# aliyun/heif-decoder-lib

Hardware: AMD Instinct MI355X
Metric: megapixels/sec HEIC grid->RGB24 (higher is better)
Workload: dtype u8

## Files before the change

### heif-decoder-lib_amd/csrc/chain.hip

```cpp
#include "recon_common.h"

#include <stdlib.h>
#include <atomic>
#include <map>
#include <memory>
#include <mutex>
#include <new>
#include <utility>

#include "hm_internal.h"

namespace {

#ifdef HM_CHAIN_TIMING
#define HM_T_DECL unsigned long long t_prev = __builtin_amdgcn_s_memtime(); unsigned int t_acc[6] = {0, 0, 0, 0, 0, 0}, t_part[4] = {0, 0, 0, 0}; int t_in_svc = 0; (void)t_part; (void)t_in_svc
#if HM_CHAIN_TIMING == 2
#define HM_T_LAP(i) (void)t_prev
#define HM_T_COUNT(i) t_acc[i] += 64
#else
#define HM_T_LAP(i) do { if (HM_CHAIN_TIMING != 4) { const unsigned long long t_now = __builtin_amdgcn_s_memtime(); t_acc[i] += (unsigned int)(t_now - t_prev); t_prev = t_now; } } while (0)
#define HM_T_COUNT(i)
#endif
#if HM_CHAIN_TIMING == 4
#define HM_T_SVC_BEGIN() do { t_prev = __builtin_amdgcn_s_memtime(); t_in_svc = 1; } while (0)
// ... 53 lines not shown
  int rows_per_wave, split_kinds, bands_per_pic;
  int passes;
  int ring;
  int spin_limit;
  int test_stall;
  int early;
};
constexpr int SYNC_TICKET = 0, SYNC_PROGRESS = 8;
constexpr int SPIN_LIMIT = 1 << 20;

__device__ __forceinline__ int g_of(int lane) { return lane >> 4; }
template <int CTRL>
__device__ __forceinline__ int dpp(int v) { return __builtin_amdgcn_update_dpp(0, v, CTRL, 0xF, 0xF, false); }
constexpr int DPP_ROW_ROR(int n) { return 0x120 | n; }
constexpr int DPP_ROW_SHR(int n) { return 0x110 | n; }

enum { ST_START = 0, ST_RUN = 1, ST_DONE = 2 };

typedef uint32_t c_u32x4 __attribute__((ext_vector_type(4)));
typedef uint32_t c_u32x2 __attribute__((ext_vector_type(2)));

#ifndef HM_WPE_ONE_CHAIN
#define HM_WPE_ONE_CHAIN 5
#endif
#ifndef HM_WPE_CTB64
#define HM_WPE_CTB64 4
#endif
template <typename Pix, int LOG2_CTB, int MODE>
constexpr int chain_waves_per_simd = (sizeof(Pix) == 1 && MODE == 0) ? (LOG2_CTB <= 5 ? 5 : HM_WPE_CTB64) :
                                     ((MODE >= 3 && !(sizeof(Pix) == 2 && LOG2_CTB == 6)) ? HM_WPE_ONE_CHAIN : 4);
// ... 519 lines not shown
      uint32_t run[2], big[2];
#pragma unroll
      for (int c = 0; c < 2; c++) {
        const uint32_t q = of_chain(gq, c), r = of_chain(gr, c);
        run[c] = (uint32_t)__builtin_ctz(~q | (1u << SUBX));
        big[c] = (uint32_t)__builtin_ctz(~((r & ~q) >> run[c]));
      }
      const uint32_t my_run = g == 0 ? run[0] : run[1], my_big = g == 0 ? big[0] : big[1];
      quad = (uint32_t)my_off < my_run;
      m_quad = ballot(quad);
      s_big = ballot((uint32_t)my_off >= my_run && (uint32_t)my_off < my_run + my_big);
      n_exec = (int)(my_run + my_big);
      n_sub = (int)(run[0] > run[1] ? run[0] : run[1]);
    }
    (void)m_quad;
    const unsigned long long s_bres = s_big & ballot((op.y & (OP_CBF | (3u << OP_L2_SHIFT))) == (OP_CBF | (1u << OP_L2_SHIFT)));

    HM_T_LAP(1);
#if defined(HM_Q_PROBE) && (HM_Q_PROBE & 2048)
    if (s_bres && n_pics < 0) {
#else
    if (s_bres) {
#endif
      auto big_res = [&](int gg) -> uint32_t {
        uint32_t idx = (uint32_t)__builtin_amdgcn_readlane((int)op.z, gg * 16) + (uint32_t)lane;
        idx = idx < res_last ? idx : res_last;
        return (uint32_t)(int)resid[idx];
      };
      uint32_t sb_lo = (uint32_t)s_bres, sb_hi = (uint32_t)(s_bres >> 32);
      asm volatile("" : "+s"(sb_lo), "+s"(sb_hi));
      if (sb_lo & 0xFFFFu) bres0 = big_res(0);
// ... 81 lines not shown
      HM_T_COUNT(4);
      const int src = bg * 16;
      const uint32_t ox = (uint32_t)__builtin_amdgcn_readlane((int)op.x, src), oy = (uint32_t)__builtin_amdgcn_readlane((int)op.y, src);
      const uint32_t oz = (uint32_t)__builtin_amdgcn_readlane((int)op.z, src), ow = (uint32_t)__builtin_amdgcn_readlane((int)op.w, src);
      const uint32_t s_gb = (uint32_t)__builtin_amdgcn_readlane((int)gb_off, src), s_tl = (uint32_t)__builtin_amdgcn_readlane((int)tl_off, src);
      const int mode = (int)(oy & OP_MODE_MASK), c = (int)((oy >> OP_C_SHIFT) & 3), log2 = 2 + (int)((oy >> OP_L2_SHIFT) & 3);
      const int path = (int)((oy >> OP_PATH_SHIFT) & 7);
#ifdef HM_D_SKIP
      if ((HM_D_SKIP >> (path != PATH_GEN ? path : 4 + log2)) & 1) continue;
#endif
#if defined(HM_Q_PROBE) && (HM_Q_PROBE & 512)
      const bool cbf = false;
#else
      const bool cbf = (oy & OP_CBF) != 0;
#endif
      const int P = c == 0 ? P0 : P1;
      Pix* const gb = reinterpret_cast<Pix*>(lds + s_gb);
      Pix* const lp = gb + (ox & 0xFFFF);
      const Pix* const tp = reinterpret_cast<const Pix*>(lds + ((oy & OP_LINE) ? s_tl : s_gb)) + (ox >> 16) + 1;
      Pix* const dst = lp + 1;
      const GLOBAL_AS int16_t* const gres = resid + oz;
      const int maxv = (1 << bd) - 1;

      HM_MARK("D_setup_end");
      auto block = [&](auto l2c, auto which) {
        constexpr int L2 = decltype(l2c)::value, WHICH = decltype(which)::value;
        int ln = lane;
        asm volatile("" : "+v"(ln));
        int res_s = 0, res_t[4] = {0, 0, 0, 0};
        const bool pairs = sizeof(Pix) == 1 && L2 >= 4 && WHICH != PATH_B4 && mode >= 2 && mode != 10 && mode != 26;
#ifdef HM_PAIRS_PRE
        uint32_t res_p[2] = {0, 0};
        if (cbf && pairs && L2 == 4) {
#pragma unroll
          for (int t = 0; t < 2; t++) res_p[t] = pairs8_residual<4>(mode >= 18, ln, t, gres);
        }
        else
#endif
        if (cbf && !pairs) {
          if (L2 == 2) {
            const int s_ri = __builtin_amdgcn_readlane((int)ri_me, src);
            const int s_chain = PAIRS ? bg & ((1 << NCL) - 1) : ((CAN_LATE && late) ? bg & 2 : bg);
            res_s = (int)(rres_all + s_chain * (RING * 16) + (s_ri & (RING - 1)) * 16)[ln & 15];
          }
          else if (L2 == 3) {
            uint32_t b = bg == 0 ? bres0 : (bg == 1 ? bres1 : (bg == 2 ? bres2 : bres3));
            asm volatile("" : "+v"(b));
            res_s = (int)b;
          }
          else if (L2 == 4) {
#pragma unroll
            for (int t = 0; t < 4; t++) res_t[t] = (int)gres[ln + 64 * t];
          }
        }
        auto emit = [&](int p, int x, int y, int v) {
          if (cbf) {
            int r;
            if (L2 <= 3) r = res_s;
            else if (L2 == 4) {
              const int t = rfl(p >> 6);
              r = t == 0 ? res_t[0] : (t == 1 ? res_t[1] : (t == 2 ? res_t[2] : res_t[3]));
            }
            else r = (int)gres[p];
            v = clip3i(0, maxv, v + r);
          }
          dst[mul24(y, P) + x] = (Pix)v;
        };
        Blk<Pix> B;
        B.mode = mode; B.c = c; B.bd = bd; B.log2 = L2; B.tskip = 0; B.qp = 0; B.n_coeff = 0; B.P = P;
        const bool smoothed = L2 != 2 && c == 0 && ((filter_mode_mask(L2) >> mode) & 1);
#if !defined(HM_Q_PROBE) || !(HM_Q_PROBE & 4)
        if (false) {}
        else if (WHICH == PATH_I16) {
// ... 3 lines not shown
          const int j = ln - 32;
          const int p = R(j), p_end = R(32);
          int pf = p;
          if (smoothed) {
            const int pm = dpp<0x138>(p);
            int pp = dpp<0x130>(p);
            pp = ln == 63 ? p_end : pp;
            pf = j == -32 ? p : (pm + 2 * p + pp + 2) >> 2;
          }
          int16_t* const bc = l_bA + 64;
          bc[j] = (int16_t)pf;
          if (ln == 0) bc[32] = (int16_t)p_end;
          WAVE_SYNC();
          if constexpr (sizeof(Pix) == 1 && L2 == 4) {
#ifdef HM_PAIRS_PRE
            if (pairs) predict_pairs8<4, true>(mode, bc, tab, ln, cbf, gres, reinterpret_cast<uint8_t*>(dst), P, res_p);
#else
            if (pairs) predict_pairs8<4, false>(mode, bc, tab, ln, cbf, gres, reinterpret_cast<uint8_t*>(dst), P);
#endif
            else predict_emit<Pix, L2>(B, RefArray{bc}, tab, ln, emit);
          }
          else predict_emit<Pix, L2>(B, RefArray{bc}, tab, ln, emit);
        }
        else if (WHICH == PATH_B4) {
          const uint32_t avail = ((ow & OPW_LEFT) ? 0xF0u : 0u) | (((ow >> OPW_BL_SHIFT) & 15) ? 0x0Fu : 0u) | ((ow & OPW_TL) ? 0x100u : 0u) |
                                 ((ow & OPW_TOP) ? 0x1E00u : 0u) | (((ow >> OPW_TR_SHIFT) & 15) ? 0x1E000u : 0u);
          const int b = ln < 16 ? ln : 16;
          const uint32_t lower = avail & ((1u << b) - 1u);
          const int first = avail ? (int)__builtin_ctz(avail) : 0;
          const int from = ((avail >> b) & 1u) ? b : (lower ? 31 - (int)__builtin_clz(lower) : first);
          const int j = from - 8;
          const Pix* const ql = lp + mul24_raw(-j - 1, P);
          const Pix* const qt = tp + (j - 1);
// ... 6 lines not shown
        }
        else {
          constexpr uint32_t nT = 1u << L2;
          B.info = L2 | (c << HM_TU_CIDX_SHIFT) | ((ow & OPW_TL) ? HM_TU_AVAIL_TL : 0);
          B.aBL = (int)(((ow >> OPW_BL_SHIFT) & 15) << 2); B.aTR = (int)(((ow >> OPW_TR_SHIFT) & 15) << 2);
          B.avail = ((ow & OPW_LEFT) ? nT : 0u) | ((uint32_t)B.aBL << 8) | ((ow & OPW_TOP) ? nT << 16 : 0u) | ((uint32_t)B.aTR << 24);
          B.x0 = (int)((ow >> 6) & 0x3C); B.y0 = (int)((ow >> 10) & 0x3C);
          B.u = gb + (c == 2 ? cr_off : 0);
          B.top = reinterpret_cast<const Pix*>(lds + s_tl) + (c == 2 ? Wc + 4 : 0);
#if !defined(HM_Q_PROBE) || !(HM_Q_PROBE & 16)
          make_border<Pix, L2>(B, l_bA, strong, ln);
          WAVE_SYNC();
          if constexpr (sizeof(Pix) == 1 && L2 >= 4) {
            if (pairs) {
#ifdef HM_PAIRS_PRE
              if constexpr (L2 == 4) predict_pairs8<4, true>(mode, l_bA + 64, tab, ln, cbf, gres, reinterpret_cast<uint8_t*>(dst), P, res_p);
              else
#endif
              predict_pairs8<L2, false>(mode, l_bA + 64, tab, ln, cbf, gres, reinterpret_cast<uint8_t*>(dst), P);
            }
            else predict_emit<Pix, L2>(B, RefArray{l_bA + 64}, tab, ln, emit);
          }
          else predict_emit<Pix, L2>(B, RefArray{l_bA + 64}, tab, ln, emit);
#endif
        }
#endif
        if (L2 >= 4) __builtin_amdgcn_s_waitcnt(0x0F70);
        WAVE_SYNC();
        HM_MARK("D_pred_end");
      };
#if defined(HM_Q_PROBE) && (HM_Q_PROBE & 256)
      if (path == PATH_F8A) continue;
#endif
#if !defined(HM_Q_PROBE) || !(HM_Q_PROBE & 128)
// ... 14 lines not shown
        }
        else {
          const int inv = inv_angle_of(mode);
          const int k0 = k + 1, k1 = k + 2;
          const int q0 = -((mul24(k0, inv) + 128) >> 8), q1 = -((mul24(k1, inv) + 128) >> 8);
          const int j0 = k0 >= 0 ? k0 : q0, j1 = k1 >= 0 ? k1 : q1;
          auto at = [&](int j, bool main_side) -> int {
            const Pix* const qm = vert ? tp + imin_(j - 1, nT1) : lp + mul24(imin_(j - 1, nL1), P);
            const Pix* const qs = vert ? lp + mul24(imin_(-j - 1, nL1), P) : tp + imin_(-j - 1, nT1);
            return *(main_side ? qm : qs);
          };
          r0 = vert ? at(j0, j0 >= 0) : at(j0, j0 > 0);
          r1 = vert ? at(j1, j1 >= 0) : at(j1, j1 > 0);
        }
        int v = blend32(f, r0, r1);
        if (cbf) {
          uint32_t b = bg == 0 ? bres0 : (bg == 1 ? bres1 : (bg == 2 ? bres2 : bres3));
          asm volatile("" : "+v"(b));
          v = clip3i(0, maxv, v + (int)b);
        }
        dst[mul24(y, P) + x] = (Pix)v;
        WAVE_SYNC();
        continue;
      }
      else if (path == PATH_F8O) {
        int ln = lane;
        asm volatile("" : "+v"(ln));
        const int x = ln & 7, y = ln >> 3;
        const int nL1 = (int)((oy >> OP_NL1_SHIFT) & 63), nT1 = (int)((oy >> OP_NT1_SHIFT) & 63);
        const int t = tp[x], l = lp[mul24(y, P)];
        int v;
        if (mode == 0) v = planar_sample<3>(x, y, l, t, tp[imin_(8, nT1)], lp[mul24(imin_(8, nL1), P)]);
        else if (mode == 1) {
          int s2 = ln < 8 ? t : (ln < 16 ? (int)lp[mul24(ln - 8, P)] : 0);
          s2 += dpp<DPP_ROW_ROR(8)>(s2);
// ... 6 lines not shown
            const int dc3 = mad24_k<3>(dc, 2);
            v = y == 0 ? (t + dc3) >> 2 : v;
            v = x == 0 ? (l + dc3) >> 2 : v;
            v = (x | y) == 0 ? (l + 2 * dc + t + 2) >> 2 : v;
          }
        }
        else {
          const bool vert = mode == 26;
          v = vert ? t : l;
          if (c == 0) {
            const int corner = tp[-1];
            const int gq = vert ? (int)tp[0] + ((l - corner) >> 1) : (int)lp[0] + ((t - corner) >> 1);
            v = (vert ? x == 0 : y == 0) ? clip3i(0, maxv, gq) : v;
          }
        }
        if (cbf) {
          uint32_t b = bg == 0 ? bres0 : (bg == 1 ? bres1 : (bg == 2 ? bres2 : bres3));
          asm volatile("" : "+v"(b));
          v = clip3i(0, maxv, v + (int)b);
        }
        dst[mul24(y, P) + x] = (Pix)v;
        WAVE_SYNC();
        continue;
      }
      else if (path == PATH_S8) {
        int ln = lane;
        asm volatile("" : "+v"(ln));
        const int nL1 = (int)((oy >> OP_NL1_SHIFT) & 63), nT1 = (int)((oy >> OP_NT1_SHIFT) & 63);
        const int j = ln < 32 ? ln - 16 : 16;
        const Pix* const ql = lp + mul24_raw(imin_(-j - 1, nL1), P);
        const Pix* const qt = tp + imin_(j - 1, nT1);
        const int p = *(j < 0 ? ql : qt);
        const int pm = dpp<0x138>(p), pp = dpp<0x130>(p);
        const int pf = (j == -16 || j == 16) ? p : (pm + 2 * p + pp + 2) >> 2;
        int16_t* const bc = l_bA + 64;
        if (ln <= 32) bc[j] = (int16_t)pf;
        WAVE_SYNC();
        const int x = ln & 7, y = ln >> 3;
        int v;
        if (mode == 0) v = planar_sample<3>(x, y, bc[-1 - y], bc[1 + x], bc[9], bc[-9]);
        else v = bc[mode == 34 ? x + y + 2 : (mode == 2 ? -(x + y + 2) : x - y)];
        if (cbf) {
          uint32_t b = bg == 0 ? bres0 : (bg == 1 ? bres1 : (bg == 2 ? bres2 : bres3));
          asm volatile("" : "+v"(b));
          v = clip3i(0, maxv, v + (int)b);
        }
        dst[mul24(y, P) + x] = (Pix)v;
        WAVE_SYNC();
        continue;
      }
#endif
#if defined(HM_Q_PROBE) && (HM_Q_PROBE & 96)
      {
        const bool sm = log2 == 3 && c == 0 && ((filter_mode_mask(3) >> mode) & 1);
        const bool fast = log2 <= 3 && !sm && (oy & OP_INTERIOR);
        if (((HM_Q_PROBE & 32) && !fast) || ((HM_Q_PROBE & 64) && fast)) continue;
      }
#endif
      typedef std::integral_constant<int, PATH_GEN> gen_t;
      if (path == PATH_I16) block(std::integral_constant<int, 4>(), std::integral_constant<int, PATH_I16>());
      else if (path == PATH_B4) block(std::integral_constant<int, 2>(), std::integral_constant<int, PATH_B4>());
// ... 550 lines not shown
```

### heif-decoder-lib_amd/csrc/recon_common.h

```cpp
#ifndef HM_RECON_COMMON_H
#define HM_RECON_COMMON_H

#include <hip/hip_runtime.h>
#include <stdint.h>
#include <type_traits>

#include "hm_device.h"

namespace {

#define WAVE_SYNC()                                          \
  do {                                                       \
    __builtin_amdgcn_fence(__ATOMIC_ACQ_REL, "wavefront");  \
    __builtin_amdgcn_wave_barrier();                         \
  } while (0)

__device__ __forceinline__ int clip3i(int lo, int hi, int v) { return v < lo ? lo : (v > hi ? hi : v); }
__device__ __forceinline__ int iabs_(int v) { return v < 0 ? -v : v; }
__device__ __forceinline__ int imin_(int a, int b) { return a < b ? a : b; }
__device__ __forceinline__ int mul24(int a, int b) { return __mul24(a, b); }
__device__ __forceinline__ int mul24_raw(int a, int b)
{
  int d;
  asm("v_mul_i32_i24 %0, %1, %2" : "=v"(d) : "v"(a), "v"(b));
// ... 58 lines not shown
  return -(int)(((ad <= 4 ? K1 : K2) >> (16 * ((ad - 1) & 3))) & 0xFFFF);
}
namespace angle_check {
constexpr int kAngle[35] = {0, 0, 32, 26, 21, 17, 13, 9, 5, 2, 0, -2, -5, -9, -13, -17, -21, -26, -32, -26, -21, -17, -13, -9, -5, -2, 0, 2, 5, 9, 13, 17, 21, 26, 32};
constexpr int kInv[15] = {-4096, -1638, -910, -630, -482, -390, -315, -256, -315, -390, -482, -630, -910, -1638, -4096};
constexpr bool same()
{
  for (int m = 2; m < 35; m++)
    if (intra_angle_of(m) != kAngle[m]) return false;
  for (int m = 11; m <= 25; m++)
    if (inv_angle_of(m) != kInv[m - 11]) return false;
  return true;
}
static_assert(same(), "intra_angle_of / inv_angle_of must reproduce Tables 8-4 / 8-5");
}
__constant__ int c_level_scale[6] = {40, 45, 51, 57, 64, 72};
__constant__ int8_t c_dst[4][4] = {{29, 55, 74, 84}, {74, 74, 0, -74}, {84, -29, -74, 55}, {55, -84, 74, -29}};
__constant__ int8_t c_dct_mag[33] = {64, 90, 90, 90, 89, 88, 87, 85, 83, 82, 80, 78, 75, 73, 70, 67, 64,
                                     61, 57, 54, 50, 46, 43, 38, 36, 31, 25, 22, 18, 13, 9, 4, 0};

#define GLOBAL_AS __attribute__((address_space(1)))
template <typename T>
__device__ __forceinline__ const GLOBAL_AS T* gptr(const void* p) { return (const GLOBAL_AS T*)(uintptr_t)p; }
template <typename T>
__device__ __forceinline__ GLOBAL_AS T* gptr_w(void* p) { return (GLOBAL_AS T*)(uintptr_t)p; }

constexpr int BIG_BYTES = 2048 + 1024 + 16;
constexpr int UPAD = 4;

template <typename Pix>
struct Blk {
  Pix* u;
  const Pix* top;
  int P;
// ... 259 lines not shown
    });
    }
  }
}
template <int L2>
__device__ __forceinline__ uint32_t pairs8_residual(bool vert, int lane, int t, const GLOBAL_AS int16_t* gres)
{
  constexpr int nT = 1 << L2;
  const int q = lane + 64 * t;
  const int x = vert ? (q & (nT / 2 - 1)) << 1 : q & (nT - 1), y = vert ? q >> (L2 - 1) : (q >> L2) << 1;
  if (vert) return *reinterpret_cast<const GLOBAL_AS uint32_t*>(gres + (x + (y << L2)));
  return (uint32_t)(uint16_t)gres[x + (y << L2)] | ((uint32_t)(uint16_t)gres[x + ((y + 1) << L2)] << 16);
}
template <int L2, bool PRE = false>
__device__ __forceinline__ void predict_pairs8(int mode, const int16_t* bc, const int16_t* tab, int lane, bool cbf, const GLOBAL_AS int16_t* gres, uint8_t* dst, int P,
                                               const uint32_t* pre = nullptr)
{
  constexpr int nT = 1 << L2, TRIPS = nT * nT / 128;
  typedef short s16x2_t __attribute__((ext_vector_type(2)));
  typedef unsigned short u16x2_t __attribute__((ext_vector_type(2)));
  const int angle = __builtin_amdgcn_readfirstlane((int)tab[mode]);
  const int inv = __builtin_amdgcn_readfirstlane((int)tab[35 + mode]);
  const bool vert = mode >= 18;
  auto ref = [&](int k) -> uint32_t {
    const int a = k >= 0 ? k : -((mul24(k, inv) + 128) >> 8);
    return (uint32_t)(uint16_t)bc[vert ? a : -a];
  };
  auto ref_pos = [&](int k) -> uint32_t { return (uint32_t)(uint16_t)bc[vert ? k : -k]; };
  auto trip = [&](int t) {
    const int q = lane + 64 * t;
    const int major = vert ? q >> (L2 - 1) : q & (nT - 1);
    const int m0 = vert ? (q & (nT / 2 - 1)) << 1 : (q >> L2) << 1;
    const int tt = mul24(major + 1, angle);
    const int k0 = m0 + (tt >> 5) + 1;
    const uint32_t f = (uint32_t)(tt & 31);
    uint32_t r0, r1, r2;
    if (angle > 0) { r0 = ref_pos(k0); r1 = ref_pos(k0 + 1); r2 = ref_pos(k0 + 2); }
    else { r0 = ref(k0); r1 = ref(k0 + 1); r2 = ref(k0 + 2); }
    const uint32_t A = r0 | (r1 << 16), B = r1 | (r2 << 16);
    const uint32_t w1 = f | (f << 16), w0 = 0x00200020u - w1;
    u16x2_t v = __builtin_bit_cast(u16x2_t, A) * __builtin_bit_cast(u16x2_t, w0) + __builtin_bit_cast(u16x2_t, B) * __builtin_bit_cast(u16x2_t, w1) + (u16x2_t)(16);
    v = v >> (u16x2_t)(5);
    const int x = vert ? m0 : major, y = vert ? major : m0;
    if (cbf) {
      uint32_t rr;
      if constexpr (PRE) rr = pre[t];
      else rr = pairs8_residual<L2>(vert, lane, t, gres);
      s16x2_t s = __builtin_bit_cast(s16x2_t, v) + __builtin_bit_cast(s16x2_t, rr);
      s = __builtin_elementwise_min(__builtin_elementwise_max(s, (s16x2_t)(0)), (s16x2_t)(255));
      v = __builtin_bit_cast(u16x2_t, s);
    }
    const uint32_t vw = __builtin_bit_cast(uint32_t, v);
    uint8_t* const o = dst + mul24(y, P) + x;
    if (vert) *reinterpret_cast<uint16_t*>(o) = (uint16_t)((vw & 0xFFu) | ((vw >> 8) & 0xFF00u));
    else { o[0] = (uint8_t)vw; o[P] = (uint8_t)(vw >> 16); }
  };
  if constexpr (TRIPS <= 2) {
#pragma unroll
    for (int t = 0; t < TRIPS; t++) trip(t);
  }
  else {
// ... 25 lines not shown
  return g;
}

constexpr uint32_t OP_MODE_MASK = 63u;
constexpr int OP_C_SHIFT = 6, OP_L2_SHIFT = 8;
constexpr uint32_t OP_CBF = 1u << 10, OP_INTERIOR = 1u << 11, OP_LINE = 1u << 13;
constexpr uint32_t OP_FAR = 1u << 26;
constexpr uint32_t OP_FAST8 = 1u << 12;
constexpr int OP_PATH_SHIFT = 27;
enum { PATH_GEN = 0,
       PATH_F8A = 1,
       PATH_F8O = 2,
       PATH_S8 = 3,
       PATH_I16 = 4,
       PATH_B4 = 5 };
constexpr uint32_t OP_SPECIAL = 1u << 31;
constexpr int OP_NL1_SHIFT = 14, OP_NT1_SHIFT = 20;
constexpr uint32_t OPW_LEFT = 1u << 16, OPW_TOP = 1u << 17, OPW_TL = 1u << 18;
constexpr int OPW_BL_SHIFT = 19, OPW_TR_SHIFT = 23;
typedef uint32_t mop_u32x4 __attribute__((ext_vector_type(4)));
__device__ __forceinline__ mop_u32x4 make_micro_op(uint32_t r0, unsigned a_left, unsigned a_top, unsigned a_tl, uint32_t aBL4, uint32_t aTR4, uint32_t qpy,
                                                   int Pk, int cr_off, int Wc, uint32_t roff)
{
  const int x4 = (int)(r0 & 15), y4 = (int)((r0 >> 4) & 15);
  const uint32_t info = (r0 >> 8) & 0xFF;
  const int l2 = (int)(info & HM_TU_LOG2_MASK), c = (int)((info >> HM_TU_CIDX_SHIFT) & 3);
  const uint32_t mode = (r0 >> 16) & OP_MODE_MASK;
  const bool cbf = (info & HM_TU_CBF) != 0;
  const int nT = 1 << l2;
  const bool left = a_left != 0, top = a_top != 0, tl = a_tl != 0;
// ... 200 lines not shown
```

### heif-decoder-lib_amd/csrc/residual.hip

```cpp
#include <cstdio>
#include <cstdlib>

#include "recon_common.h"
#include "hm_avail.h"

#include "hm_internal.h"

namespace {

constexpr int R_WAVES = 4;
constexpr int R_TABLES_SMALL = 1024 + 256 + 128;
constexpr int R_STAGE = 256;
constexpr int R_WAVE = 2048 + 1024 + 4 * 16 * 4 + R_STAGE * 4;

template <int CTRL>
__device__ __forceinline__ int rdpp(int v) { return __builtin_amdgcn_update_dpp(0, v, CTRL, 0xF, 0xF, false); }
constexpr int R_ROW_ROR(int n) { return 0x120 | n; }
constexpr int R_QUAD_BCAST(int k) { return k | (k << 2) | (k << 4) | (k << 6); }

typedef short r_s16x2 __attribute__((ext_vector_type(2)));
typedef uint32_t r_u32x4 __attribute__((ext_vector_type(4)));
typedef uint32_t r_u32x2 __attribute__((ext_vector_type(2)));
__device__ __forceinline__ int rdot2(uint32_t a, uint32_t b, int acc)
{
// ... 13 lines not shown
  v += rdpp_m<0x114, 0xF>(v);
  v += rdpp_m<0x118, 0xF>(v);
  v += rdpp_m<0x142, 0xA>(v);
  v += rdpp_m<0x143, 0xC>(v);
  return v;
}

template <int L2>
struct BigGeom {
  static constexpr int nT = 1 << L2;
  static constexpr int MT_STRIDE = nT + 4;
};
constexpr int R_MT16 = 16 * BigGeom<4>::MT_STRIDE * 2, R_MT32 = 32 * BigGeom<5>::MT_STRIDE * 2;
constexpr int R_TABLES = R_TABLES_SMALL + R_MT16 + R_MT32;
static_assert(R_TABLES % 16 == 0, "the waves' blocks are read 16 bytes at a time");
__device__ __forceinline__ int wave_max3(int v)
{
  int m = 0;
#pragma unroll
  for (int b = 2; b >= 0; b--) {
    const int t = m | (1 << b);
    if (ballot(v >= t)) m = t;
  }
  return m;
}
template <int L2, typename Levels>
__device__ __forceinline__ void big_residual(int16_t* coeff, int16_t* tmp, const int16_t* mt, const int16_t* tab, Levels cf,
                                             int n_coeff, int qP, int bit_depth, GLOBAL_AS int16_t* __restrict__ out, int lane)
{
  constexpr int nT = 1 << L2, log2 = L2, MS = BigGeom<L2>::MT_STRIDE;
// ... 60 lines not shown
#define HM_R_WPE 7
#endif
#ifndef HM_R_SKIP
#define HM_R_SKIP 0
#endif
#define HM_R_ATTR __attribute__((amdgpu_waves_per_eu(HM_R_WPE, HM_R_WPE)))
__global__ __launch_bounds__(R_WAVES * 64) HM_R_ATTR void k_residual(const hm_dev_pic* __restrict__ pics, int n_pics, int max_ctb_h, int segs)
{
  extern __shared__ __attribute__((aligned(16))) uint8_t lds[];
  const int tid = threadIdx.x, lane = tid & 63, wave = rfl(tid >> 6);
  int8_t* const dct = reinterpret_cast<int8_t*>(lds);
  int16_t* const tab = reinterpret_cast<int16_t*>(lds + 1024);
  uint32_t* const w8 = reinterpret_cast<uint32_t*>(lds + 1024 + 256);
  int16_t* const mt16 = reinterpret_cast<int16_t*>(lds + R_TABLES_SMALL);
  int16_t* const mt32 = reinterpret_cast<int16_t*>(lds + R_TABLES_SMALL + R_MT16);
  for (int i = tid; i < 1024; i += R_WAVES * 64) {
    const int k = i >> 5, n = i & 31;
    const int m = (k * (2 * n + 1)) & 127;
    int v;
    if (k == 0) v = 64;
    else if (m <= 32) v = c_dct_mag[m];
    else if (m <= 64) v = -c_dct_mag[64 - m];
    else if (m <= 96) v = -c_dct_mag[m - 64];
    else v = c_dct_mag[128 - m];
    dct[i] = (int8_t)v;
  }
  for (int i = tid; i < 92; i += R_WAVES * 64) {
    int v = 0;
    if (i >= 70 && i < 76) v = c_level_scale[i - 70];
    else if (i >= 76) v = c_dst[(i - 76) >> 2][(i - 76) & 3];
    tab[i] = (int16_t)v;
  }
  uint8_t* const wbase = lds + R_TABLES + (size_t)wave * R_WAVE;
  int16_t* const coeff = reinterpret_cast<int16_t*>(wbase);
  int16_t* const tmp = reinterpret_cast<int16_t*>(wbase + 2048);
  int* const slots = reinterpret_cast<int*>(wbase + 2048 + 1024);
  uint32_t* const lvl = reinterpret_cast<uint32_t*>(wbase + 2048 + 1024 + 4 * 16 * 4);
  for (int i = lane; i < 1024; i += 64) coeff[i] = 0;
  slots[lane] = 0;
  __syncthreads();
  for (int t = tid; t < 32; t += R_WAVES * 64) {
    const int i = t >> 2, k = t & 3;
    w8[t] = ((uint32_t)(uint16_t)(int16_t)dct[(4 * (2 * k)) * 32 + i]) | ((uint32_t)(uint16_t)(int16_t)dct[(4 * (2 * k + 1)) * 32 + i] << 16);
  }
  for (int t = tid; t < 256 + 1024; t += R_WAVES * 64) {
    const bool big = t >= 256;
    const int u = big ? t - 256 : t, i = big ? u >> 5 : u >> 4, j = big ? u & 31 : u & 15;
    (big ? mt32 + i * BigGeom<5>::MT_STRIDE : mt16 + i * BigGeom<4>::MT_STRIDE)[j] = (int16_t)dct[((big ? 1 : 2) * j) * 32 + i];
  }
  __syncthreads();

  const uint32_t unit = (uint32_t)blockIdx.x * R_WAVES + (uint32_t)wave;
  const uint32_t per_pic = 2u * (uint32_t)max_ctb_h * (uint32_t)segs;
  const int pic_index = (int)(unit / per_pic);
  if (pic_index >= n_pics) return;
  const int rem = (int)(unit - (uint32_t)pic_index * per_pic);
  const int seg = rem % segs, rk = rem / segs;
  const int row = rk >> 1, kind = rk & 1;
  const hm_dev_pic dp = pics[pic_index];
  if (row >= dp.ctb_h || (kind && dp.chroma_format == 0)) return;
  const int x0 = (int)((long)seg * dp.ctb_w / segs), x1 = (int)((long)(seg + 1) * dp.ctb_w / segs);
  if (x0 >= x1) return;
  const uint8_t* blob = dp.blob;
  const GLOBAL_AS hm_pic* H = gptr<hm_pic>(blob);
// ... 76 lines not shown
    const int info = (int)((r0 >> 8) & 0xFF), l2 = info & HM_TU_LOG2_MASK;
    mop_u32x4 mop = {r0, 0u, 0u, 0u};
    if (!(HM_R_SKIP & 64)) {
      const int lw = k_lw, lh = k_lh;
      const int nT = 1 << l2;
      const int xin = x4 << 2, yc = k_row_y0 + (y4 << 2);
      const int ctb_pw = k_ctb_pw, rem_last = k_rem_last;
      const int room_x = (cnt_raw & HM_TU6_LAST_COLUMN) ? rem_last - (xin + nT) : ((info & HM_TU6_NEXT_TO_LAST) ? ctb_pw + rem_last - (xin + nT) : nT);
      const int room_y = k_plane_h - (yc + nT);
      const hm_avail av = hm_derive_avail(xin << lw, (y4 << 2) << lh, nT << lw, nT << lh, nT, room_x, room_y, dp.log2_ctb, (cnt_raw >> HM_TU6_NB_SHIFT) & 15u);
      mop = make_micro_op(r0, av.left, av.top, av.tl, (uint32_t)av.n_bl >> 2, (uint32_t)av.n_tr >> 2, 0u, m_Pk, m_cr_off, m_Wc, 0u);
      if (y4 == 0 && xin + nT + (int)(((uint32_t)av.n_tr >> 2) << 2) > ctb_pw) mop.y |= OP_FAR;
      asm volatile("" : "+v"(mop.x), "+v"(mop.y), "+v"(mop.w));
    }
    const bool cbf = valid && (info & HM_TU_CBF);
    const uint32_t rsz = (cbf && l2 >= 3) ? 16u << (2 * (l2 - 2)) : 0u;
    const uint32_t sc = wave_scan(cnt), sr = wave_scan(rsz);
    const uint32_t lo = lev_base + sc - cnt, ro = res_base + sr - rsz;
    mop.z = ro;
    const uint32_t n_lev = (uint32_t)__builtin_amdgcn_readlane((int)sc, 63);
    lev_base += n_lev;
    res_base += (uint32_t)__builtin_amdgcn_readlane((int)sr, 63);
    auto level = [&](uint32_t first, uint32_t i) -> uint32_t {
      const uint32_t rel = first - chunk_lev + i;
      uint32_t v;
      if (rel < (uint32_t)R_STAGE) v = lvl[rel];
      else {
        v = coeffs[first + i];
        asm volatile("" : "+v"(v));
      }
      return v;
    };
    __builtin_amdgcn_s_waitcnt(0x0F70);
#pragma unroll
    for (int k = 0; k < R_STAGE / 64; k++) lvl[lane + 64 * k] = staged[k];
    cur_x = ahead.x; cur_y = ahead.y;
    asm volatile("" : "+v"(cur_x), "+v"(cur_y));
    if (valid) mops[ri] = mop;
    if (kind == 0 && !(HM_R_SKIP & 32)) {
      if (cand_ok) {
        const uint32_t tf = cand_first - chunk;
        if (tf < 64u) __hip_atomic_fetch_add(slots + tf, 1, __ATOMIC_RELAXED, __HIP_MEMORY_SCOPE_WAVEFRONT);
      }
      WAVE_SYNC();
      int sm = slots[lane];
      WAVE_SYNC();
      slots[lane] = 0;
      sm = (int)wave_scan((uint32_t)sm);
      const int my_ctb = cur_ctb + sm;
      cur_ctb += __builtin_amdgcn_readlane(sm, 63);
      int lane_flags = __builtin_amdgcn_ds_bpermute((sm & 63) << 2, (int)ctb_flags);
      asm volatile("" : "+v"(lane_flags));
// ... 18 lines not shown
      }
      for (unsigned long long mb = ballot(valid && l2 >= 4); mb; mb &= mb - 1) {
        const int b = (int)__builtin_ctzll(mb);
        const int s_l2 = __builtin_amdgcn_readlane(l2, b), s_gx = __builtin_amdgcn_readlane(gx, b), s_gy = __builtin_amdgcn_readlane(gy, b);
        const int s_left = __builtin_amdgcn_readlane(left_ok, b), s_top = __builtin_amdgcn_readlane(top_ok, b);
        const uint32_t s_q = (uint32_t)__builtin_amdgcn_readlane((int)qword, b);
        const int n4 = 1 << (s_l2 - 2);
        const int i = lane & (n4 - 1), j = lane >> (s_l2 - 2);
        if (lane < n4 * n4 && s_gx + i < w4 && s_gy + j < h4)
          meta[(uint32_t)(s_gx + i) + __umul24((uint32_t)(s_gy + j), (uint32_t)w4)] = (uint16_t)((i == 0 ? s_left : 0) | ((j == 0 ? s_top : 0) << 1) | s_q);
      }
    }

    WAVE_SYNC();

    const uint32_t first_level = cbf ? level(lo, 0) : 0xFFFFu;
    const bool dc_only = cbf && cnt == 1 && (first_level & 0xFFFF) == 0 && !(info & HM_TU_TSKIP);
    auto dequant = [&](uint32_t raw, int qP, int l2b) -> int {
      const int q6 = (qP * 43) >> 8, qr = qP - 6 * q6;
      const int bdShift = bd + l2b - 9;
      const int32_t fact = (int32_t)tab[70 + qr] << q6;
      const int32_t prod = (int32_t)((uint32_t)mul24((int)(int16_t)(raw >> 16), fact) + (uint32_t)(1 << (bdShift - 1)));
      return clip3i(-32768, 32767, prod >> bdShift);
    };
    for (unsigned long long m4 = (HM_R_SKIP & 1) ? 0 : ballot(dc_only && l2 == 2); m4;) {
      int b[4];
#pragma unroll
      for (int k = 0; k < 4; k++) {
        b[k] = m4 ? (int)__builtin_ctzll(m4) : -1;
        m4 &= m4 - 1;
      }
      const int myb = g == 0 ? b[0] : (g == 1 ? b[1] : (g == 2 ? b[2] : b[3]));
      const bool act = myb >= 0;
      const int src = act ? myb : 0;
      const uint32_t br0 = (uint32_t)__shfl((int)r0, src), braw = (uint32_t)__shfl((int)first_level, src);
      const int c = dequant(braw, (int)(br0 >> 24), 2);
      const int m0y = kind ? 64 : (int)tab[76 + by_], m0x = kind ? 64 : (int)tab[76 + bx_];
      const int t1 = clip3i(-32768, 32767, (mul24(m0y, c) + 64) >> 7);
      int res = (mul24(m0x, t1) + rnd2) >> postShift;
      if (kind == 0) res = clip3i(-32768, 32767, res);
      if (act) res4[(size_t)(chunk + (uint32_t)myb) * 16 + (uint32_t)gl] = limit_res(res, maxv);
    }
    for (unsigned long long mdc = (HM_R_SKIP & 2) ? 0 : ballot(dc_only && l2 >= 3); mdc; mdc &= mdc - 1) {
      const int b = (int)__builtin_ctzll(mdc);
      const uint32_t s_r0 = (uint32_t)__builtin_amdgcn_readlane((int)r0, b), s_raw = (uint32_t)__builtin_amdgcn_readlane((int)first_level, b);
      const uint32_t s_ro = (uint32_t)__builtin_amdgcn_readlane((int)ro, b);
      const int s_l2 = (int)((s_r0 >> 8) & HM_TU_LOG2_MASK);
      const int c = dequant(s_raw, (int)(s_r0 >> 24), s_l2);
      const int t1 = clip3i(-32768, 32767, (64 * c + 64) >> 7);
      const int16_t k16 = limit_res((64 * t1 + rnd2) >> postShift, maxv);
      const uint32_t pair = (uint32_t)(uint16_t)k16 * 0x10001u;
      const int n_words = 1 << (2 * s_l2 - 1);
      GLOBAL_AS uint32_t* const out = reinterpret_cast<GLOBAL_AS uint32_t*>(resid + s_ro);
      for (int w = lane; w < n_words; w += 64) out[w] = pair;
    }

    for (unsigned long long m4 = (HM_R_SKIP & 4) ? 0 : ballot(cbf && l2 == 2 && !dc_only); m4;) {
      int b[4];
#pragma unroll
      for (int k = 0; k < 4; k++) {
        b[k] = m4 ? (int)__builtin_ctzll(m4) : -1;
        m4 &= m4 - 1;
      }
      const int myb = g == 0 ? b[0] : (g == 1 ? b[1] : (g == 2 ? b[2] : b[3]));
      const bool act = myb >= 0;
      const int src = act ? myb : 0;
      const uint32_t br0 = (uint32_t)__shfl((int)r0, src), bcnt = (uint32_t)__shfl((int)cnt, src);
      const uint32_t blo = (uint32_t)__shfl((int)lo, src);
      const bool has = act && (uint32_t)gl < bcnt;
      uint32_t raw = 0;
      if (has) raw = level(blo, (uint32_t)gl);
// ... 102 lines not shown
```

Baseline: 153,700.

## Pass DC-only residual constants inline via op flag instead of filling buffers

For DC-only transform units of size 8x8 and larger, the residual stage now computes the constant residual value and stores it directly in the op word with a new OP_RCONST flag. It no longer allocates and fills a residual buffer in global memory. The reconstruction chain reads the constant instead of loading residual arrays, which removes global stores and loads for those blocks. Separately, the DCT and quantisation tables are now built at compile time into a constant array and copied to LDS, replacing the runtime table-generation loops and one barrier. The trade-off is extra branches in the prediction paths and one more op-field bit to keep consistent across both kernels.

After: 155,000 (median of 6 runs). No clear change (+0.8%).

```diff
diff --git a/heif-decoder-lib_amd/csrc/chain.hip b/heif-decoder-lib_amd/csrc/chain.hip
--- a/heif-decoder-lib_amd/csrc/chain.hip
+++ b/heif-decoder-lib_amd/csrc/chain.hip
@@ -91,6 +91,13 @@
 __device__ __forceinline__ int dpp(int v) { return __builtin_amdgcn_update_dpp(0, v, CTRL, 0xF, 0xF, false); }
 constexpr int DPP_ROW_ROR(int n) { return 0x120 | n; }
 constexpr int DPP_ROW_SHR(int n) { return 0x110 | n; }
+__device__ __forceinline__ int res8(bool rconst, int rk, int bg, uint32_t b0, uint32_t b1, uint32_t b2, uint32_t b3)
+{
+  if (rconst) return rk;
+  uint32_t b = bg == 0 ? b0 : (bg == 1 ? b1 : (bg == 2 ? b2 : b3));
+  asm volatile("" : "+v"(b));
+  return (int)b;
+}
 
 enum { ST_START = 0, ST_RUN = 1, ST_DONE = 2 };
 
@@ -640,7 +647,7 @@
       n_sub = (int)(run[0] > run[1] ? run[0] : run[1]);
     }
     (void)m_quad;
-    const unsigned long long s_bres = s_big & ballot((op.y & (OP_CBF | (3u << OP_L2_SHIFT))) == (OP_CBF | (1u << OP_L2_SHIFT)));
+    const unsigned long long s_bres = s_big & ballot((op.y & (OP_CBF | OP_RCONST | (3u << OP_L2_SHIFT))) == (OP_CBF | (1u << OP_L2_SHIFT)));
 
     HM_T_LAP(1);
 #if defined(HM_Q_PROBE) && (HM_Q_PROBE & 2048)
@@ -752,6 +759,9 @@
 #else
       const bool cbf = (oy & OP_CBF) != 0;
 #endif
+      const bool rconst = (oy & OP_RCONST) != 0;
+      const int rk = (int)(int16_t)oz;
+      const uint32_t rpair = (oz & 0xFFFFu) * 0x10001u;
       const int P = c == 0 ? P0 : P1;
       Pix* const gb = reinterpret_cast<Pix*>(lds + s_gb);
       Pix* const lp = gb + (ox & 0xFFFF);
@@ -769,7 +779,7 @@
         const bool pairs = sizeof(Pix) == 1 && L2 >= 4 && WHICH != PATH_B4 && mode >= 2 && mode != 10 && mode != 26;
 #ifdef HM_PAIRS_PRE
         uint32_t res_p[2] = {0, 0};
-        if (cbf && pairs && L2 == 4) {
+        if (cbf && pairs && L2 == 4 && !rconst) {
 #pragma unroll
           for (int t = 0; t < 2; t++) res_p[t] = pairs8_residual<4>(mode >= 18, ln, t, gres);
         }
@@ -781,10 +791,11 @@
             const int s_chain = PAIRS ? bg & ((1 << NCL) - 1) : ((CAN_LATE && late) ? bg & 2 : bg);
             res_s = (int)(rres_all + s_chain * (RING * 16) + (s_ri & (RING - 1)) * 16)[ln & 15];
           }
-          else if (L2 == 3) {
-            uint32_t b = bg == 0 ? bres0 : (bg == 1 ? bres1 : (bg == 2 ? bres2 : bres3));
-            asm volatile("" : "+v"(b));
-            res_s = (int)b;
+          else if (L2 == 3) res_s = res8(rconst, rk, bg, bres0, bres1, bres2, bres3);
+          else if (rconst) {
+            res_s = rk;
+#pragma unroll
+            for (int t = 0; t < 4; t++) res_t[t] = rk;
           }
           else if (L2 == 4) {
 #pragma unroll
@@ -794,7 +805,7 @@
         auto emit = [&](int p, int x, int y, int v) {
           if (cbf) {
             int r;
-            if (L2 <= 3) r = res_s;
+            if (L2 <= 3 || (L2 == 5 && rconst)) r = res_s;
             else if (L2 == 4) {
               const int t = rfl(p >> 6);
               r = t == 0 ? res_t[0] : (t == 1 ? res_t[1] : (t == 2 ? res_t[2] : res_t[3]));
@@ -828,9 +839,9 @@
           WAVE_SYNC();
           if constexpr (sizeof(Pix) == 1 && L2 == 4) {
 #ifdef HM_PAIRS_PRE
-            if (pairs) predict_pairs8<4, true>(mode, bc, tab, ln, cbf, gres, reinterpret_cast<uint8_t*>(dst), P, res_p);
+            if (pairs) predict_pairs8<4, true>(mode, bc, tab, ln, cbf, gres, reinterpret_cast<uint8_t*>(dst), P, rconst, rpair, res_p);
 #else
-            if (pairs) predict_pairs8<4, false>(mode, bc, tab, ln, cbf, gres, reinterpret_cast<uint8_t*>(dst), P);
+            if (pairs) predict_pairs8<4, false>(mode, bc, tab, ln, cbf, gres, reinterpret_cast<uint8_t*>(dst), P, rconst, rpair);
 #endif
             else predict_emit<Pix, L2>(B, RefArray{bc}, tab, ln, emit);
           }
@@ -867,10 +878,10 @@
           if constexpr (sizeof(Pix) == 1 && L2 >= 4) {
             if (pairs) {
 #ifdef HM_PAIRS_PRE
-              if constexpr (L2 == 4) predict_pairs8<4, true>(mode, l_bA + 64, tab, ln, cbf, gres, reinterpret_cast<uint8_t*>(dst), P, res_p);
+              if constexpr (L2 == 4) predict_pairs8<4, true>(mode, l_bA + 64, tab, ln, cbf, gres, reinterpret_cast<uint8_t*>(dst), P, rconst, rpair, res_p);
               else
 #endif
-              predict_pairs8<L2, false>(mode, l_bA + 64, tab, ln, cbf, gres, reinterpret_cast<uint8_t*>(dst), P);
+              predict_pairs8<L2, false>(mode, l_bA + 64, tab, ln, cbf, gres, reinterpret_cast<uint8_t*>(dst), P, rconst, rpair);
             }
             else predict_emit<Pix, L2>(B, RefArray{l_bA + 64}, tab, ln, emit);
           }
@@ -915,11 +926,7 @@
           r1 = vert ? at(j1, j1 >= 0) : at(j1, j1 > 0);
         }
         int v = blend32(f, r0, r1);
-        if (cbf) {
-          uint32_t b = bg == 0 ? bres0 : (bg == 1 ? bres1 : (bg == 2 ? bres2 : bres3));
-          asm volatile("" : "+v"(b));
-          v = clip3i(0, maxv, v + (int)b);
-        }
+        if (cbf) v = clip3i(0, maxv, v + res8(rconst, rk, bg, bres0, bres1, bres2, bres3));
         dst[mul24(y, P) + x] = (Pix)v;
         WAVE_SYNC();
         continue;
@@ -956,11 +963,7 @@
             v = (vert ? x == 0 : y == 0) ? clip3i(0, maxv, gq) : v;
           }
         }
-        if (cbf) {
-          uint32_t b = bg == 0 ? bres0 : (bg == 1 ? bres1 : (bg == 2 ? bres2 : bres3));
-          asm volatile("" : "+v"(b));
-          v = clip3i(0, maxv, v + (int)b);
-        }
+        if (cbf) v = clip3i(0, maxv, v + res8(rconst, rk, bg, bres0, bres1, bres2, bres3));
         dst[mul24(y, P) + x] = (Pix)v;
         WAVE_SYNC();
         continue;
@@ -982,11 +985,7 @@
         int v;
         if (mode == 0) v = planar_sample<3>(x, y, bc[-1 - y], bc[1 + x], bc[9], bc[-9]);
         else v = bc[mode == 34 ? x + y + 2 : (mode == 2 ? -(x + y + 2) : x - y)];
-        if (cbf) {
-          uint32_t b = bg == 0 ? bres0 : (bg == 1 ? bres1 : (bg == 2 ? bres2 : bres3));
-          asm volatile("" : "+v"(b));
-          v = clip3i(0, maxv, v + (int)b);
-        }
+        if (cbf) v = clip3i(0, maxv, v + res8(rconst, rk, bg, bres0, bres1, bres2, bres3));
         dst[mul24(y, P) + x] = (Pix)v;
         WAVE_SYNC();
         continue;
diff --git a/heif-decoder-lib_amd/csrc/recon_common.h b/heif-decoder-lib_amd/csrc/recon_common.h
--- a/heif-decoder-lib_amd/csrc/recon_common.h
+++ b/heif-decoder-lib_amd/csrc/recon_common.h
@@ -96,10 +96,13 @@
 }
 static_assert(same(), "intra_angle_of / inv_angle_of must reproduce Tables 8-4 / 8-5");
 }
-__constant__ int c_level_scale[6] = {40, 45, 51, 57, 64, 72};
-__constant__ int8_t c_dst[4][4] = {{29, 55, 74, 84}, {74, 74, 0, -74}, {84, -29, -74, 55}, {55, -84, 74, -29}};
-__constant__ int8_t c_dct_mag[33] = {64, 90, 90, 90, 89, 88, 87, 85, 83, 82, 80, 78, 75, 73, 70, 67, 64,
-                                     61, 57, 54, 50, 46, 43, 38, 36, 31, 25, 22, 18, 13, 9, 4, 0};
+#define HM_LEVEL_SCALE 40, 45, 51, 57, 64, 72
+#define HM_DST4 {29, 55, 74, 84}, {74, 74, 0, -74}, {84, -29, -74, 55}, {55, -84, 74, -29}
+#define HM_DCT_MAG 64, 90, 90, 90, 89, 88, 87, 85, 83, 82, 80, 78, 75, 73, 70, 67, 64, \
+                   61, 57, 54, 50, 46, 43, 38, 36, 31, 25, 22, 18, 13, 9, 4, 0
+__constant__ int c_level_scale[6] = {HM_LEVEL_SCALE};
+__constant__ int8_t c_dst[4][4] = {HM_DST4};
+__constant__ int8_t c_dct_mag[33] = {HM_DCT_MAG};
 
 #define GLOBAL_AS __attribute__((address_space(1)))
 template <typename T>
@@ -389,7 +392,7 @@
 }
 template <int L2, bool PRE = false>
 __device__ __forceinline__ void predict_pairs8(int mode, const int16_t* bc, const int16_t* tab, int lane, bool cbf, const GLOBAL_AS int16_t* gres, uint8_t* dst, int P,
-                                               const uint32_t* pre = nullptr)
+                                               bool rconst, uint32_t rpair, const uint32_t* pre = nullptr)
 {
   constexpr int nT = 1 << L2, TRIPS = nT * nT / 128;
   typedef short s16x2_t __attribute__((ext_vector_type(2)));
@@ -419,7 +422,8 @@
     const int x = vert ? m0 : major, y = vert ? major : m0;
     if (cbf) {
       uint32_t rr;
-      if constexpr (PRE) rr = pre[t];
+      if (rconst) rr = rpair;
+      else if constexpr (PRE) rr = pre[t];
       else rr = pairs8_residual<L2>(vert, lane, t, gres);
       s16x2_t s = __builtin_bit_cast(s16x2_t, v) + __builtin_bit_cast(s16x2_t, rr);
       s = __builtin_elementwise_min(__builtin_elementwise_max(s, (s16x2_t)(0)), (s16x2_t)(255));
@@ -475,6 +479,7 @@
        PATH_S8 = 3,
        PATH_I16 = 4,
        PATH_B4 = 5 };
+constexpr uint32_t OP_RCONST = 1u << 30;
 constexpr uint32_t OP_SPECIAL = 1u << 31;
 constexpr int OP_NL1_SHIFT = 14, OP_NT1_SHIFT = 20;
 constexpr uint32_t OPW_LEFT = 1u << 16, OPW_TOP = 1u << 17, OPW_TL = 1u << 18;
diff --git a/heif-decoder-lib_amd/csrc/residual.hip b/heif-decoder-lib_amd/csrc/residual.hip
--- a/heif-decoder-lib_amd/csrc/residual.hip
+++ b/heif-decoder-lib_amd/csrc/residual.hip
@@ -51,6 +51,34 @@
 constexpr int R_MT16 = 16 * BigGeom<4>::MT_STRIDE * 2, R_MT32 = 32 * BigGeom<5>::MT_STRIDE * 2;
 constexpr int R_TABLES = R_TABLES_SMALL + R_MT16 + R_MT32;
 static_assert(R_TABLES % 16 == 0, "the waves' blocks are read 16 bytes at a time");
+struct alignas(16) RTables { uint8_t b[R_TABLES]; };
+constexpr int r_dct(int k, int n)
+{
+  constexpr int8_t mag[33] = {HM_DCT_MAG};
+  const int m = (k * (2 * n + 1)) & 127;
+  return k == 0 ? 64 : (m <= 32 ? mag[m] : (m <= 64 ? -mag[64 - m] : (m <= 96 ? -mag[m - 64] : mag[128 - m])));
+}
+constexpr RTables make_rtables()
+{
+  constexpr int level_scale[6] = {HM_LEVEL_SCALE};
+  constexpr int8_t dst[4][4] = {HM_DST4};
+  RTables t{};
+  auto put16 = [&t](int off, int v) { t.b[off] = (uint8_t)(v & 0xFF); t.b[off + 1] = (uint8_t)((v >> 8) & 0xFF); };
+  for (int i = 0; i < 1024; i++) t.b[i] = (uint8_t)(r_dct(i >> 5, i & 31) & 0xFF);
+  for (int i = 0; i < 6; i++) put16(1024 + 2 * (70 + i), level_scale[i]);
+  for (int i = 0; i < 16; i++) put16(1024 + 2 * (76 + i), dst[i >> 2][i & 3]);
+  for (int w = 0; w < 32; w++) {
+    const int i = w >> 2, k = w & 3;
+    put16(1024 + 256 + 4 * w, r_dct(4 * (2 * k), i));
+    put16(1024 + 256 + 4 * w + 2, r_dct(4 * (2 * k + 1), i));
+  }
+  for (int i = 0; i < 16; i++)
+    for (int j = 0; j < 16; j++) put16(R_TABLES_SMALL + 2 * (i * BigGeom<4>::MT_STRIDE + j), r_dct(2 * j, i));
+  for (int i = 0; i < 32; i++)
+    for (int j = 0; j < 32; j++) put16(R_TABLES_SMALL + R_MT16 + 2 * (i * BigGeom<5>::MT_STRIDE + j), r_dct(j, i));
+  return t;
+}
+__constant__ RTables c_rtables = make_rtables();
 __device__ __forceinline__ int wave_max3(int v)
 {
   int m = 0;
@@ -141,22 +169,9 @@
   uint32_t* const w8 = reinterpret_cast<uint32_t*>(lds + 1024 + 256);
   int16_t* const mt16 = reinterpret_cast<int16_t*>(lds + R_TABLES_SMALL);
   int16_t* const mt32 = reinterpret_cast<int16_t*>(lds + R_TABLES_SMALL + R_MT16);
-  for (int i = tid; i < 1024; i += R_WAVES * 64) {
-    const int k = i >> 5, n = i & 31;
-    const int m = (k * (2 * n + 1)) & 127;
-    int v;
-    if (k == 0) v = 64;
-    else if (m <= 32) v = c_dct_mag[m];
-    else if (m <= 64) v = -c_dct_mag[64 - m];
-    else if (m <= 96) v = -c_dct_mag[m - 64];
-    else v = c_dct_mag[128 - m];
-    dct[i] = (int8_t)v;
-  }
-  for (int i = tid; i < 92; i += R_WAVES * 64) {
-    int v = 0;
-    if (i >= 70 && i < 76) v = c_level_scale[i - 70];
-    else if (i >= 76) v = c_dst[(i - 76) >> 2][(i - 76) & 3];
-    tab[i] = (int16_t)v;
+  if (!(HM_R_SKIP & 128)) {
+    const r_u32x4* const src = reinterpret_cast<const r_u32x4*>(c_rtables.b);
+    for (int i = tid; i < R_TABLES / 16; i += R_WAVES * 64) reinterpret_cast<r_u32x4*>(lds)[i] = src[i];
   }
   uint8_t* const wbase = lds + R_TABLES + (size_t)wave * R_WAVE;
   int16_t* const coeff = reinterpret_cast<int16_t*>(wbase);
@@ -165,16 +180,6 @@
   uint32_t* const lvl = reinterpret_cast<uint32_t*>(wbase + 2048 + 1024 + 4 * 16 * 4);
   for (int i = lane; i < 1024; i += 64) coeff[i] = 0;
   slots[lane] = 0;
-  __syncthreads();
-  for (int t = tid; t < 32; t += R_WAVES * 64) {
-    const int i = t >> 2, k = t & 3;
-    w8[t] = ((uint32_t)(uint16_t)(int16_t)dct[(4 * (2 * k)) * 32 + i]) | ((uint32_t)(uint16_t)(int16_t)dct[(4 * (2 * k + 1)) * 32 + i] << 16);
-  }
-  for (int t = tid; t < 256 + 1024; t += R_WAVES * 64) {
-    const bool big = t >= 256;
-    const int u = big ? t - 256 : t, i = big ? u >> 5 : u >> 4, j = big ? u & 31 : u & 15;
-    (big ? mt32 + i * BigGeom<5>::MT_STRIDE : mt16 + i * BigGeom<4>::MT_STRIDE)[j] = (int16_t)dct[((big ? 1 : 2) * j) * 32 + i];
-  }
   __syncthreads();
 
   const uint32_t unit = (uint32_t)blockIdx.x * R_WAVES + (uint32_t)wave;
@@ -281,13 +286,10 @@
       asm volatile("" : "+v"(mop.x), "+v"(mop.y), "+v"(mop.w));
     }
     const bool cbf = valid && (info & HM_TU_CBF);
-    const uint32_t rsz = (cbf && l2 >= 3) ? 16u << (2 * (l2 - 2)) : 0u;
-    const uint32_t sc = wave_scan(cnt), sr = wave_scan(rsz);
-    const uint32_t lo = lev_base + sc - cnt, ro = res_base + sr - rsz;
-    mop.z = ro;
+    const uint32_t sc = wave_scan(cnt);
+    const uint32_t lo = lev_base + sc - cnt;
     const uint32_t n_lev = (uint32_t)__builtin_amdgcn_readlane((int)sc, 63);
     lev_base += n_lev;
-    res_base += (uint32_t)__builtin_amdgcn_readlane((int)sr, 63);
     auto level = [&](uint32_t first, uint32_t i) -> uint32_t {
       const uint32_t rel = first - chunk_lev + i;
       uint32_t v;
@@ -303,6 +305,30 @@
     for (int k = 0; k < R_STAGE / 64; k++) lvl[lane + 64 * k] = staged[k];
     cur_x = ahead.x; cur_y = ahead.y;
     asm volatile("" : "+v"(cur_x), "+v"(cur_y));
+    WAVE_SYNC();
+
+    const uint32_t first_level = cbf ? level(lo, 0) : 0xFFFFu;
+    const bool dc_only = cbf && cnt == 1 && (first_level & 0xFFFF) == 0 && !(info & HM_TU_TSKIP);
+    auto dequant = [&](uint32_t raw, int qP, int l2b) -> int {
+      const int q6 = (qP * 43) >> 8, qr = qP - 6 * q6;
+      const int bdShift = bd + l2b - 9;
+      const int32_t fact = (int32_t)tab[70 + qr] << q6;
+      const int32_t prod = (int32_t)((uint32_t)mul24((int)(int16_t)(raw >> 16), fact) + (uint32_t)(1 << (bdShift - 1)));
+      return clip3i(-32768, 32767, prod >> bdShift);
+    };
+    const bool rconst = dc_only && l2 >= 3;
+    uint32_t rk = 0;
+    if (rconst && !(HM_R_SKIP & 2)) {
+      const int c = dequant(first_level, (int)(r0 >> 24), l2);
+      const int t1 = clip3i(-32768, 32767, (64 * c + 64) >> 7);
+      rk = (uint32_t)(uint16_t)limit_res((64 * t1 + rnd2) >> postShift, maxv);
+    }
+    const uint32_t rsz = (cbf && l2 >= 3 && !rconst) ? 16u << (2 * (l2 - 2)) : 0u;
+    const uint32_t sr = wave_scan(rsz);
+    const uint32_t ro = res_base + sr - rsz;
+    res_base += (uint32_t)__builtin_amdgcn_readlane((int)sr, 63);
+    mop.z = rconst ? rk : ro;
+    mop.y |= rconst ? OP_RCONST : 0u;
     if (valid) mops[ri] = mop;
     if (kind == 0 && !(HM_R_SKIP & 32)) {
       if (cand_ok) {
@@ -351,15 +377,6 @@
 
     WAVE_SYNC();
 
-    const uint32_t first_level = cbf ? level(lo, 0) : 0xFFFFu;
-    const bool dc_only = cbf && cnt == 1 && (first_level & 0xFFFF) == 0 && !(info & HM_TU_TSKIP);
-    auto dequant = [&](uint32_t raw, int qP, int l2b) -> int {
-      const int q6 = (qP * 43) >> 8, qr = qP - 6 * q6;
-      const int bdShift = bd + l2b - 9;
-      const int32_t fact = (int32_t)tab[70 + qr] << q6;
-      const int32_t prod = (int32_t)((uint32_t)mul24((int)(int16_t)(raw >> 16), fact) + (uint32_t)(1 << (bdShift - 1)));
-      return clip3i(-32768, 32767, prod >> bdShift);
-    };
     for (unsigned long long m4 = (HM_R_SKIP & 1) ? 0 : ballot(dc_only && l2 == 2); m4;) {
       int b[4];
 #pragma unroll
@@ -378,20 +395,6 @@
       if (kind == 0) res = clip3i(-32768, 32767, res);
       if (act) res4[(size_t)(chunk + (uint32_t)myb) * 16 + (uint32_t)gl] = limit_res(res, maxv);
     }
-    for (unsigned long long mdc = (HM_R_SKIP & 2) ? 0 : ballot(dc_only && l2 >= 3); mdc; mdc &= mdc - 1) {
-      const int b = (int)__builtin_ctzll(mdc);
-      const uint32_t s_r0 = (uint32_t)__builtin_amdgcn_readlane((int)r0, b), s_raw = (uint32_t)__builtin_amdgcn_readlane((int)first_level, b);
-      const uint32_t s_ro = (uint32_t)__builtin_amdgcn_readlane((int)ro, b);
-      const int s_l2 = (int)((s_r0 >> 8) & HM_TU_LOG2_MASK);
-      const int c = dequant(s_raw, (int)(s_r0 >> 24), s_l2);
-      const int t1 = clip3i(-32768, 32767, (64 * c + 64) >> 7);
-      const int16_t k16 = limit_res((64 * t1 + rnd2) >> postShift, maxv);
-      const uint32_t pair = (uint32_t)(uint16_t)k16 * 0x10001u;
-      const int n_words = 1 << (2 * s_l2 - 1);
-      GLOBAL_AS uint32_t* const out = reinterpret_cast<GLOBAL_AS uint32_t*>(resid + s_ro);
-      for (int w = lane; w < n_words; w += 64) out[w] = pair;
-    }
-
     for (unsigned long long m4 = (HM_R_SKIP & 4) ? 0 : ballot(cbf && l2 == 2 && !dc_only); m4;) {
       int b[4];
 #pragma unroll
```
